# maxrmorrison/promonet

Hardware: AMD Instinct MI355X
Metric: audio samples/sec (22.05 kHz), batch-32 10 s utterances (higher is better)
Workload: dtype bf16; 1 GPU; Generator.forward (prepare_features + HiFi-GAN), batch 32 x 10 s per GPU (861 frames, 220416 samples each), random-init weights, bf16 MFMA operands, fp32 accumulate and activations; model=hifigan, batch_per_gpu=32, frames=861, devices=1, parallelism=batch-sharded x1

## Files before the change

include/promonet_hip.h:

```cpp
#ifndef PROMONET_HIP_H
#define PROMONET_HIP_H

#include <stddef.h>
#include <stdint.h>

#ifdef __cplusplus
extern "C" {
#endif

#define PM_OK 0
#define PM_EINVAL (-1)
#define PM_ESTATE (-2)
#define PM_EHIP (-3)
#define PM_ENOMEM (-4)
#define PM_ETIMEOUT (-5)

#define PM_F32 0
#define PM_F16 1
#define PM_BF16 2
#define PM_F16X3 3
#define PM_F16A2 4
#define PM_F16UX 5

#define PM_MAX_STAGES 8
// ... 100 lines not shown
                          int mode, float scale, void* workspace,
                          size_t workspace_bytes, void* stream);
int pm_block_cl(int dtype, const float* x_cl, float* out_cl,
                const float* const* w1, const float* const* b1,
                const float* const* w2, const float* const* b2,
                const int* dilations, int niter, int batch, int length,
                int channels, int kernel_size, int mode, float scale,
                void* workspace, size_t workspace_bytes, void* stream);
int pm_block_act16_cl(int dtype, int act_dtype, const float* x_cl,
                      float* out_cl, void* act16_cl, const float* const* w1,
                      const float* const* b1, const float* const* w2,
                      const float* const* b2, const int* dilations, int niter,
                      int batch, int length, int channels, int kernel_size,
                      int mode, float scale, void* workspace,
                      size_t workspace_bytes, void* stream);
int pm_mrf_cl(int dtype, const float* x_cl, float* out_cl,
              const float* const* w1, const float* const* b1,
              const float* const* w2, const float* const* b2,
              const int* dilations, int niter, int batch, int length,
              int channels, void* workspace, size_t workspace_bytes,
              void* stream);
int pm_input_conv_cl(int dtype, const float* x_cl, float* out_cl,
                     const float* weight, const float* bias,
                     const float* global_features,
                     const float* speaker_weight, const float* speaker_bias,
                     int global_batch, int global_channels, int batch,
                     int length, int c_in, int c_out, void* workspace,
                     size_t workspace_bytes, void* stream);
int pm_conv_transpose_cl(int dtype, const float* x_cl, float* out_cl,
                         const float* w, const float* bias, int batch,
                         int length, int c_in, int c_out, int rate, int lrelu,
                         void* workspace, size_t workspace_bytes,
                         void* stream);
int pm_conv_transpose_x16_cl(int dtype, const void* x16_cl, float* out_cl,
                             const float* w, const float* bias, int batch,
                             int length, int c_in, int c_out, int rate,
                             void* workspace, size_t workspace_bytes,
                             void* stream);
int pm_out_conv_tanh(const float* x_cl, const float* w, float* out,
                     int batch, int length, int channels, void* stream);
int pm_debug_timeline(void* dev_buffer);
int pm_debug_force(int walk_nseg, int upsample_groups);
int pm_debug_skew(int mode);
int pm_mfma_probe(int dtype, int iterations, const void* operands,
                  float* sink, int workgroups, void* stream);
size_t pm_walk_scratch_bytes(int batch);
int pm_fold_weight_norm(const float* g, const float* v, float* w, int rows,
                        int cols, void* stream);
int pm_to_channels_last(const float* src, float* dst, int batch, int channels,
                        int frames, int c_pad, void* stream);

int pm_grid_sample(const float* seq, const float* grid, float* out, int rows,
                   int n_in, int n_out, int mode, float scale, float offset,
                   float lo, float hi, void* stream);
int pm_stretch_grid(const float* ppg, int ppg_rows, const int* indices,
                    int n_indices, float* selected, float* grid, int frames,
                    int target_frames, void* stream);

#define PM_FARGAN_MIXED 16
typedef struct pm_fargan_s* pm_fargan_t;
int pm_fargan_create(int num_features, int global_channels, int weight_dtype,
                     pm_fargan_t* out);
int pm_fargan_destroy(pm_fargan_t h);
int pm_fargan_load_tensor(pm_fargan_t h, const char* name, const float* dev,
                          const int64_t* shape, int ndim, void* stream);
int pm_fargan_finalize(pm_fargan_t h, void* stream);
// ... 281 lines not shown
```

promonet_amd/_lib.py:

```python
import ctypes
import os
from pathlib import Path

import torch

LIB_PATH = Path(__file__).parent / 'lib' / 'libpromonet_hip.so'

PM_F32, PM_F16, PM_BF16, PM_F16X3, PM_F16A2, PM_F16UX = 0, 1, 2, 3, 4, 5
DTYPES = {'fp32': PM_F32, 'f32': PM_F32, 'f16': PM_F16, 'fp16': PM_F16,
          'bf16': PM_BF16, 'f16x3': PM_F16X3, 'f16a2': PM_F16A2,
          'f16ux': PM_F16UX,
          'mixed': 16}
MAX_STAGES, MAX_RESBLOCKS, MAX_DILATIONS = 8, 4, 4
SPARSE_METHODS = {None: 0, 'percentile': 1, 'constant': 2, 'topk': 3}
DISC_SPEC_R, DISC_SPEC_CMB, DISC_SPEC_DB = range(3)
FDISC_ACTIVATIONS = {'none': 0, 'relu': 1, 'sigmoid': 2}
(ADV_ABS_DIFF, ADV_SQ_ONE_MINUS, ADV_SQ, ADV_HINGE_ONE_MINUS,
 ADV_HINGE_ONE_PLUS) = range(5)
(OPTIM_MAX, OPTIM_MIN, OPTIM_MEAN, OPTIM_NORM, OPTIM_NORM_SQ, OPTIM_NONFINITE,
 OPTIM_FOUND_INF, OPTIM_INV_SCALE, OPTIM_COEF) = range(9)
OPTIM_STATS = 16

c_float_p = ctypes.c_void_p
c_int64_p = ctypes.POINTER(ctypes.c_int64)
# ... 21 lines not shown
    'pm_version': (_I, []),
    'pm_last_error': (ctypes.c_char_p, []),
    'pm_hifigan_create': (_I, [ctypes.POINTER(HifiganConfig),
                               ctypes.POINTER(_P)]),
    'pm_hifigan_destroy': (_I, [_P]),
    'pm_hifigan_load_tensor': (_I, [_P, ctypes.c_char_p, _P, c_int64_p, _I, _P]),
    'pm_hifigan_finalize': (_I, [_P, _P]),
    'pm_hifigan_workspace_bytes': (_S, [_P, _I, _I]),
    'pm_hifigan_hopsize': (_I, [_P]),
    'pm_hifigan_features_cl_channels': (_I, [_P]),
    'pm_hifigan_forward': (_I, [_P, _P, _P, _I, _P, _I, _I, _P, _S, _P]),
    'pm_hifigan_forward_cl': (_I, [_P, _P, _P, _I, _P, _I, _I, _P, _S, _P]),
    'pm_hifigan_forward_ragged': (_I, [_P, _P, _I, _P, _I, _P, _P, _I, _I, _P, _S, _P]),
    'pm_hifigan_context': (_I, [_P, ctypes.POINTER(_I), ctypes.POINTER(_I)]),
    'pm_hifigan_stream': (_I, [_P, _P, _I, _I, _P, _I, _I, _P, _P, _I, _I, _I,
                               _P, _I, _P, _S, _P]),
    'pm_hifigan_stream_workspace_bytes': (_S, [_P, _I, _I]),
    'pm_hifigan_profile_enable': (_I, [_P, _I]),
    'pm_hifigan_profile_only': (_I, [_P, ctypes.c_char_p]),
    'pm_hifigan_profile_collect': (_I, [_P]),
    'pm_hifigan_profile_reset': (_I, [_P]),
    'pm_hifigan_profile_report': (ctypes.c_char_p, [_P]),
    'pm_prepare_features': (_I, [_P] * 8 + [_I] * 9 + [_F] * 6 + [_P]),
    'pm_prepare_global_features': (_I, [_P] * 5 + [_I, _I, _I, _P]),
    'pm_prepare_global_features_linear': (_I, [_P] * 6 + [_I, _I, _I, _P]),
    'pm_op_workspace_bytes': (_S, [_I, _I, _I]),
    'pm_block_iteration_cl': (_I, [_I] + [_P] * 6 + [_I] * 6 + [_F, _P, _S, _P]),
    'pm_block_cl': (_I, [_I, _P, _P] + [_P] * 5 + [_I] * 6 + [_F, _P, _S, _P]),
    'pm_block_act16_cl': (
        _I, [_I, _I, _P, _P, _P] + [_P] * 5 + [_I] * 6 + [_F, _P, _S, _P]),
    'pm_mrf_cl': (_I, [_I, _P, _P] + [_P] * 5 + [_I] * 4 + [_P, _S, _P]),
    'pm_input_conv_cl': (_I, [_I] + [_P] * 7 + [_I] * 6 + [_P, _S, _P]),
    'pm_conv_transpose_cl': (_I, [_I] + [_P] * 4 + [_I] * 6 + [_P, _S, _P]),
    'pm_conv_transpose_x16_cl': (_I, [_I] + [_P] * 4 + [_I] * 5 + [_P, _S, _P]),
    'pm_out_conv_tanh': (_I, [_P, _P, _P, _I, _I, _I, _P]),
    'pm_debug_timeline': (_I, [_P]),
    'pm_debug_force': (_I, [_I, _I]),
    'pm_debug_skew': (_I, [_I]),
    'pm_mfma_probe': (_I, [_I, _I, _P, _P, _I, _P]),
    'pm_walk_scratch_bytes': (_S, [_I]),
    'pm_fold_weight_norm': (_I, [_P, _P, _P, _I, _I, _P]),
    'pm_to_channels_last': (_I, [_P, _P, _I, _I, _I, _I, _P]),
    'pm_grid_sample': (_I, [_P, _P, _P, _I, _I, _I, _I, _F, _F, _F, _F, _P]),
    'pm_stretch_grid': (_I, [_P, _I, _P, _I, _P, _P, _I, _I, _P]),
    'pm_fargan_create': (_I, [_I, _I, _I, ctypes.POINTER(_P)]),
    'pm_fargan_destroy': (_I, [_P]),
    'pm_fargan_load_tensor': (_I, [_P, ctypes.c_char_p, _P, c_int64_p, _I, _P]),
    'pm_fargan_finalize': (_I, [_P, _P]),
    'pm_fargan_workspace_bytes': (_S, [_P, _I, _I]),
    'pm_fargan_forward': (_I, [_P, _P, _I, _P, _I, _P, _I, _P, _I, _I, _P, _S, _P]),
    'pm_fargan_forward_ragged': (_I, [_P, _P, _I, _P, _I, _P, _I, _P, _P, _I, _I, _P, _S, _P]),
    'pm_fargan_forward_stateful': (_I, [_P, _P, _I, _P, _I, _P, _I, _P, _P, _P, _P, _I, _I, _P, _S, _P]),
    'pm_fargan_set_mode': (_I, [_P, _I]),
    'pm_fargan_check': (_I, [_P, _I, _I, _P, _P]),
    'pm_stft_scratch_bytes': (_S, [_I, _I]),
    'pm_stft_magnitude': (_I, [_P, _P, _I, _I, _P, _S, _P]),
    'pm_stft_magnitude_dft': (_I, [_P, _P, _I, _I, _P, _S, _P]),
    'pm_stft_mel_scratch_bytes': (_S, [_I]),
    'pm_stft_mel_prepare': (_I, [_P, _I, _P, _S, _P]),
    'pm_stft_mel': (_I, [_P, _P, _P, _I, _I, _I, _I, _F, _P]),
    'pm_stft_set_frames_per_group': (_I, [_I]),
    'pm_stft_set_loudness_passes': (_I, [_I]),
    'pm_stft_launch_info': (_I, [_I, _I, _I, ctypes.POINTER(_I), ctypes.POINTER(_I)]),
    'pm_linear_to_mel': (_I, [_P, _P, _P, _I, _I, _I, _I, _I, _F, _P]),
    'pm_stft_backward_scratch_bytes': (_S, [_I, _I]),
    'pm_stft_magnitude_backward': (_I, [_P, _P, _P, _I, _I, _P, _S, _P]),
# ... 137 lines not shown
```

promonet_amd/csrc/pm_api.hip:

```cpp
#include <hip/hip_runtime.h>

#include <algorithm>
#include <cstdarg>
#include <cstdio>
#include <cstring>
#include <map>
#include <mutex>
#include <string>
#include <vector>

#include "pm_host.h"
#include "pm_launch.h"
#include "pm_misc.h"

#define PM_VERSION 100

static thread_local char g_error[512] = "";

int pm_fail(int code, const char* fmt, ...) {
    va_list ap;
    va_start(ap, fmt);
    vsnprintf(g_error, sizeof(g_error), fmt, ap);
    va_end(ap);
    return code;
// ... 1187 lines not shown
    if (!x || !out || !w || !bias || !global || !ws_w || !ws_b || !ws)
        return pm_fail(PM_EINVAL, "null argument");
    if (gbatch != 1 && gbatch != B)
        return pm_fail(PM_EINVAL, "global batch must be 1 or batch");
    const int cop = pm_pad32(c_out);
    if (cop % 64 && cop != 32)
        return pm_fail(PM_EINVAL, "output channels %d unsupported", c_out);
    const InputConvLayout l = input_conv_layout(c_in, c_out, B, ws);
    if (ws_bytes < l.total)
        return pm_fail(PM_ENOMEM, "workspace too small");
    hipStream_t s = (hipStream_t)stream;
    Layer conv = input_layer(dtype, c_in, c_out);
    conv.w = l.w; conv.bias = l.bias;
    PM_HIP_TRY(pack_layer(conv, w, bias, s));
    PM_HIP_TRY(launch_speaker_bias(global, ws_w, ws_b, l.gbias, gbatch, G,
                                   c_out, s));
    PM_HIP_TRY(launch_input_conv(conv, x, out, l.gbias, gbatch, B, L, nullptr,
                                 s));
    return PM_OK;
}

struct TransposeLayout { float *w, *bias; size_t total; };
static TransposeLayout transpose_layout(int c_in, int c_out, int r,
                                        void* base) {
    const size_t ci = pm_pad32(c_in), co = pm_pad32(c_out);
    PmCarve c(base);
    float* w = c.take<float>(ci * co * 2 * r);
    c.take<float>(ci * co * 2 * r);
    return {w, c.take<float>(co * r), c.used};
}

static int conv_transpose_cl_impl(
    int dtype, const float* x, const void* x16, float* out, const float* w,
    const float* bias, int B, int L, int c_in, int c_out, int r, int lrelu,
    void* ws, size_t ws_bytes, void* stream) {
    if ((!x && !x16) || !out || !w || !bias || !ws)
        return pm_fail(PM_EINVAL, "null argument");
    if (r < 2 || (r & 1)) return pm_fail(PM_EINVAL, "rate %d unsupported", r);
    if (ws_bytes < pm_op_workspace_bytes(c_in, c_out, 2 * r))
        return pm_fail(PM_ENOMEM, "workspace too small");
    const TransposeLayout l = transpose_layout(c_in, c_out, r, ws);
    if (l.total > pm_op_workspace_bytes(c_in, c_out, 2 * r))
        return pm_fail(PM_ESTATE, "the layout outgrew its public bound");
    hipStream_t s = (hipStream_t)stream;
    Layer up = upsample_layer(dtype, c_in, c_out, r);
    if (x16 && !takes_x16(up))
        return pm_fail(PM_EINVAL, "a 16-bit operand input needs a 16-bit "
                       "operand type and the narrow upsampler kernel");
    up.w = l.w; up.bias = l.bias;
    PM_HIP_TRY(pack_layer(up, w, bias, s));
    PM_HIP_TRY(launch_upsample(up, x, x16, out, lrelu, B, L, nullptr, 1, s));
    return PM_OK;
}

extern "C" int pm_conv_transpose_cl(
    int dtype, const float* x, float* out, const float* w, const float* bias,
    int B, int L, int c_in, int c_out, int r, int lrelu, void* ws,
    size_t ws_bytes, void* stream) {
    if (!x) return pm_fail(PM_EINVAL, "null argument");
    return conv_transpose_cl_impl(dtype, x, nullptr, out, w, bias, B, L, c_in,
                                  c_out, r, lrelu, ws, ws_bytes, stream);
}

extern "C" int pm_conv_transpose_x16_cl(
    int dtype, const void* x16, float* out, const float* w, const float* bias,
    int B, int L, int c_in, int c_out, int r, void* ws, size_t ws_bytes,
    void* stream) {
    if (!x16) return pm_fail(PM_EINVAL, "null argument");
    return conv_transpose_cl_impl(dtype, nullptr, x16, out, w, bias, B, L, c_in,
                                  c_out, r, 1, ws, ws_bytes, stream);
}

extern "C" int pm_out_conv_tanh(
    const float* x, const float* w, float* out, int B, int L, int C,
    void* stream) {
    if (!x || !w || !out) return pm_fail(PM_EINVAL, "null argument");
    if (pm_pad32(C) > 64)
        return pm_fail(PM_EINVAL, "channels %d unsupported", C);
    PM_HIP_TRY(launch_out_conv(x, w, out, B, L, C, nullptr, 1,
                               (hipStream_t)stream));
    return PM_OK;
}

static bool debug_hooks_enabled() {
    static const bool enabled = [] {
        const char* e = getenv("PROMONET_HIP_DEBUG");
        return e && e[0] == '1';
    }();
    return enabled;
}

extern "C" int pm_debug_force(int walk_nseg, int upsample_groups) {
    if (!debug_hooks_enabled())
        return pm_fail(PM_ESTATE, "debug hooks are disabled "
                       "(start the process with PROMONET_HIP_DEBUG=1)");
    if (walk_nseg < 0 || upsample_groups < 0)
        return pm_fail(PM_EINVAL, "negative value");
    pm_force().walk_nseg = walk_nseg;
    pm_force().upsample_groups = upsample_groups;
    return PM_OK;
}

extern "C" int pm_mfma_probe(int dtype, int iterations, const void* operands,
// ... 92 lines not shown
```

promonet_amd/csrc/pm_common.h:

```cpp
#pragma once
#include <hip/hip_runtime.h>
#include <stdint.h>

#define PM_LRELU_SLOPE 0.1f

typedef float floatx16 __attribute__((ext_vector_type(16)));
typedef unsigned int pm_u4 __attribute__((ext_vector_type(4)));
typedef _Float16 half8 __attribute__((ext_vector_type(8)));
typedef _Float16 half4 __attribute__((ext_vector_type(4)));
typedef __bf16 bf16x8 __attribute__((ext_vector_type(8)));
typedef __bf16 bf16x4 __attribute__((ext_vector_type(4)));

__device__ __forceinline__ float pm_lrelu(float v) {
    return __builtin_fmaxf(v, v * PM_LRELU_SLOPE);
}
typedef float pm_f4 __attribute__((ext_vector_type(4)));
__device__ __forceinline__ float4 pm_lrelu4(float4 v) {
    pm_f4 w = {v.x, v.y, v.z, v.w};
    w = __builtin_elementwise_max(w, w * PM_LRELU_SLOPE);
    return make_float4(w.x, w.y, w.z, w.w);
}

#define PM_ELEM_COMMON(bias_split)                                            \
    static constexpr bool BIAS_SPLIT = bias_split;                            \
// ... 196 lines not shown
    typedef ElemF16X3::frag_t bfrag_t;
    typedef afrag_t frag_t;
    static constexpr int ESZ = 4;
    static constexpr int WSZ = 2;
    static constexpr int ID = 4;
    static constexpr bool SPLIT = true;
    static constexpr bool BIAS_SPLIT = true;
    __device__ static __forceinline__ void mma(
        const afrag_t& a, const bfrag_t& b, floatx16& c) {
        c = __builtin_amdgcn_mfma_f32_32x32x16_f16(a, b.lo, c, 0, 0, 0);
        c = __builtin_amdgcn_mfma_f32_32x32x16_f16(a, b.hi, c, 0, 0, 0);
    }
    __device__ static __forceinline__ void store4_at(
        char* rowp, int ch, float4 v) {
        ElemF16X3::store4_at(rowp, ch, v);
    }
    __device__ static __forceinline__ void pack_store(
        void* out, long long index, float v) {
        reinterpret_cast<_Float16*>(out)[index] = (_Float16)v;
    }
    __device__ static __forceinline__ lds_t cvt(float v) { return (_Float16)v; }
    __device__ static __forceinline__ void mma_bias(
        const afrag_t& a, floatx16& c) {
        ElemF16::mma_bias(a, c);
    }
};

__device__ __forceinline__ void pm_block_sync() {
    __builtin_amdgcn_fence(__ATOMIC_RELEASE, "workgroup", "local");
    __builtin_amdgcn_s_barrier();
    __builtin_amdgcn_fence(__ATOMIC_ACQUIRE, "workgroup", "local");
}

__device__ __forceinline__ int pm_xcd_remap(int bid, int nwg) {
    const int xcd = bid & 7;
    const int q = nwg >> 3, r = nwg & 7;
    const int base = xcd < r ? xcd * (q + 1) : r * (q + 1) + (xcd - r) * q;
    return base + (bid >> 3);
}
```

promonet_amd/csrc/pm_conv.h:

```cpp
#pragma once
#include <type_traits>

#include "pm_common.h"


template <class ET, int CH, int NT, int XR_MAX>
struct ChunkStager {
    static constexpr int Q = CH / 4;
    static constexpr int MAXIT = (XR_MAX * Q + NT - 1) / NT;
    static constexpr int S = CH * ET::ESZ + 16;
    float4 r[MAXIT];

    __device__ __forceinline__ void load(
        const float* __restrict__ xb, int cstride, int c0, int t_first,
        int XR, int L, int tid) {
        const int lo = max(t_first, 0);
        const int hi = min(L, t_first + XR);
        const __amdgpu_buffer_rsrc_t rsrc = __builtin_amdgcn_make_buffer_rsrc(
            const_cast<float*>(xb) + (size_t)lo * cstride, 0,
            max(hi - lo, 0) * cstride * 4, 0x00020000);
#pragma unroll
        for (int it = 0; it < MAXIT; ++it) {
            const int idx = tid + it * NT;
            const int row = idx / Q, q = idx % Q;
// ... 597 lines not shown
                                              acc[mt][nt][4 * g4 + 2] * scale);
                        r.w = __float_as_uint(__uint_as_float(o.w) +
                                              acc[mt][nt][4 * g4 + 3] * scale);
                        __builtin_amdgcn_raw_buffer_store_b128(
                            r, orsrc, voff + g4 * 32, 0, 0);
                    }
                }
            }
    } else {
        const float s = mode == 1 ? scale : 1.f;
#pragma unroll
        for (int mt = 0; mt < MTW; ++mt)
#pragma unroll
            for (int nt = 0; nt < NTW; ++nt) {
                const unsigned voff =
                    voff0 + (unsigned)((mt * 32 + nt * 32 * C) * 4);
#pragma unroll
                for (int g4 = 0; g4 < 4; ++g4) {
                    pm_u4 r;
                    r.x = __float_as_uint(acc[mt][nt][4 * g4 + 0] * s);
                    r.y = __float_as_uint(acc[mt][nt][4 * g4 + 1] * s);
                    r.z = __float_as_uint(acc[mt][nt][4 * g4 + 2] * s);
                    r.w = __float_as_uint(acc[mt][nt][4 * g4 + 3] * s);
                    __builtin_amdgcn_raw_buffer_store_b128(
                        r, orsrc, voff + g4 * 32, 0, 0);
                }
            }
    }
    PM_STAMP(a, 5);
    PM_STAMP_WALL(a, blockIdx.x, 13);
}


struct SingleArgs {
    const void* x16;
    const float* x;
    float* out;
    const void* w;
    const float* bias;
    const float* gbias;
    int gbias_batch;
    int B, L, Cin, M;
    int Lout;
    int bins;
    unsigned* maxbits;
    const float* grad;
    int lrelu;
    int pad;
    int phase_c, phase_p, phase_r;
    int ntiles, nmblocks;
    const int* lengths;
    int len_scale;
};

__device__ __forceinline__ unsigned pm_float_order_bits(float f) {
    const unsigned u = __float_as_uint(f);
    return (u & 0x80000000u) ? ~u : (u | 0x80000000u);
}

template <class ET, int KT, int KSPAN, int CH, int WM, int WN, int MTW, int NTW,
          int EPI>
__global__ __launch_bounds__(WM * WN * 64) void conv_single_kernel(
    SingleArgs a) {
    typedef typename ET::afrag_t frag_t;
    constexpr int KC = CH / 16;
    constexpr int N1 = WN * NTW * 32;
// ... 57 lines not shown
    const frag_t* w = reinterpret_cast<const frag_t*>(a.w) +
                      (size_t)(m0 / 32) * w_mt_stride + lane;
    frag_t afirst[G][MTW];
    load_a_group<ET, MTW, G>(afirst, w, w_mt_stride);
    const int lane_off_x =
        ((wn * NTW * 32) + ln + js) * SX + lh * 8 * ET::ESZ;

#pragma unroll 1
    for (int c = 0; c < NCH; ++c) {
        char* cur = smem + (c & 1) * XR * SX;
        if (c + 1 < NCH) {
            if (pre) stager.load16(xb16, Cin, (c + 1) * CH, t_first, XR, L, tid);
            else stager.load(xb, Cin, (c + 1) * CH, t_first, XR, L, tid);
        }
        mma_taps<ET, KT, KC, MTW, NTW, G, SX>(
            acc, cur + lane_off_x, SX, w + (size_t)c * (KT * KC * 64),
            w_mt_stride, afirst,
            c + 1 < NCH ? w + (size_t)(c + 1) * (KT * KC * 64) : nullptr);
        if (c + 1 < NCH) {
            char* nxt = smem + ((c + 1) & 1) * XR * SX;
            if (pre) stager.store16(nxt, XR, tid);
            else if (a.lrelu) stager.template store<true>(nxt, XR, tid);
            else stager.template store<false>(nxt, XR, tid);
            pm_block_sync();
        }
    }

    if constexpr (EPI == 0) {
    const float* gb = a.gbias
        ? a.gbias + (size_t)(a.gbias_batch == 1 ? 0 : b) * M : nullptr;
    const __amdgpu_buffer_rsrc_t orsrc = __builtin_amdgcn_make_buffer_rsrc(
        a.out + ((size_t)b * a.Lout + t0) * M, 0,
        min(Lout - t0, N1) * M * 4, 0x00020000);
#pragma unroll
    for (int mt = 0; mt < MTW; ++mt) {
        const int co_base = m0 + mt * 32 + 4 * lh;
        float4 bias[4];
#pragma unroll
        for (int g4 = 0; g4 < 4; ++g4) {
            const int co = co_base + 8 * g4;
            bias[g4] = *reinterpret_cast<const float4*>(a.bias + co);
            if (gb) {
                const float4 g = *reinterpret_cast<const float4*>(gb + co);
                bias[g4].x += g.x; bias[g4].y += g.y;
                bias[g4].z += g.z; bias[g4].w += g.w;
            }
        }
#pragma unroll
        for (int nt = 0; nt < NTW; ++nt) {
            const int n = (wn * NTW + nt) * 32 + ln;
            const unsigned voff = (unsigned)((n * M + co_base) * 4);
#pragma unroll
            for (int g4 = 0; g4 < 4; ++g4) {
                pm_u4 r;
                r.x = __float_as_uint(acc[mt][nt][4 * g4 + 0] + bias[g4].x);
                r.y = __float_as_uint(acc[mt][nt][4 * g4 + 1] + bias[g4].y);
                r.z = __float_as_uint(acc[mt][nt][4 * g4 + 2] + bias[g4].z);
                r.w = __float_as_uint(acc[mt][nt][4 * g4 + 3] + bias[g4].w);
                __builtin_amdgcn_raw_buffer_store_b128(
                    r, orsrc, voff + g4 * 32, 0, 0);
            }
        }
    }
    } else if constexpr (EPI == 3) {
    float* ob = a.out + (size_t)b * a.Lout * M;
    const float* gb = a.grad + (size_t)b * a.bins * a.Lout;
#pragma unroll
    for (int mt = 0; mt < MTW; ++mt) {
        const int row_base = m0 + mt * 32 + 4 * lh;
#pragma unroll
        for (int nt = 0; nt < NTW; ++nt) {
            const int n = (wn * NTW + nt) * 32 + ln;
            const int t = t0 + n;
            if (t < a.Lout) {
#pragma unroll
                for (int g4 = 0; g4 < 4; ++g4) {
                    float v[4];
#pragma unroll
                    for (int pr = 0; pr < 2; ++pr) {
                        const int bin = (row_base + 8 * g4) / 2 + pr;
                        const float re = acc[mt][nt][4 * g4 + 2 * pr];
                        const float im = acc[mt][nt][4 * g4 + 2 * pr + 1];
                        float scale = 0.f;
                        if (bin < a.bins)
                            scale = gb[(size_t)bin * a.Lout + t] /
                                    sqrtf(re * re + im * im + 1e-6f);
                        v[2 * pr] = scale * re;
                        v[2 * pr + 1] = scale * im;
                    }
                    *reinterpret_cast<float4*>(
                        ob + (size_t)t * M + row_base + 8 * g4) =
                        make_float4(v[0], v[1], v[2], v[3]);
                }
            }
        }
// ... 10 lines not shown
            const int t = t0 + n;
#pragma unroll
            for (int g4 = 0; g4 < 4; ++g4) {
#pragma unroll
                for (int pr = 0; pr < 2; ++pr) {
                    const int bin = (row_base + 8 * g4) / 2 + pr;
                    const float re = acc[mt][nt][4 * g4 + 2 * pr];
                    const float im = acc[mt][nt][4 * g4 + 2 * pr + 1];
                    const float pw = re * re + im * im;
                    if (t < a.Lout && bin < a.bins) {
                        float v;
                        if constexpr (EPI == 1) {
                            v = sqrtf(pw + 1e-6f);
                        } else {
                            v = 10.f * log10f(fmaxf(1e-10f, pw));
                            local_max = fmaxf(local_max, v);
                        }
                        ob[(size_t)bin * a.Lout + t] = v;
                    }
                }
            }
        }
    }
    if constexpr (EPI == 2) {
#pragma unroll
        for (int o = 32; o > 0; o >>= 1)
            local_max = fmaxf(local_max, __shfl_xor(local_max, o, 64));
        if (lane == 0 && local_max > -INFINITY)
            atomicMax(a.maxbits + b, pm_float_order_bits(local_max));
    }
    }
}

template <class ET, int CIN, int WM, int WN, int MTW, int NTW>
__global__ __launch_bounds__(WM * WN * 64) void conv_upsample_kernel(
    SingleArgs a) {
    typedef typename ET::afrag_t frag_t;
    constexpr int KT = 2, KSPAN = 3;
    constexpr int KC = CIN / 16;
    constexpr int N1 = WN * NTW * 32;
    constexpr int NT = WM * WN * 64;
    constexpr int S = CIN * ET::ESZ + 16;
    constexpr int XR = N1 + KSPAN - 1;
    constexpr int MB = WM * MTW * 32;
    constexpr int G = 4;
    constexpr int SLAB = 128;

    extern __shared__ __attribute__((aligned(16))) char smem[];

    const int tid = threadIdx.x;
    const int lane = tid & 63;
    const int wave = __builtin_amdgcn_readfirstlane(tid >> 6);
    const int wm = wave / WN, wn = wave % WN;
    const int ln = lane & 31, lh = lane >> 5;

    const int wg = pm_xcd_remap(blockIdx.x, gridDim.x);
    const int mg = wg % a.nmblocks;
    const int tile = (wg / a.nmblocks) % a.ntiles;
    const int b = wg / (a.nmblocks * a.ntiles);
    const int t0 = tile * N1;
    const int M = a.M;
    const int L = a.lengths ? min(a.lengths[b] * a.len_scale, a.L) : a.L;
    const int Lout = a.lengths ? L : a.Lout;
    if (t0 >= Lout) return;

    const float* xb = a.x + (size_t)b * a.L * CIN;
    const int t_first = t0 - a.pad;
// ... 12 lines not shown

    constexpr int w_mt_stride = KT * KC * 64;
    const int per_group = (M / MB) / a.nmblocks;
    const frag_t* wbase = reinterpret_cast<const frag_t*>(a.w) + lane;
    const float* gb = a.gbias
        ? a.gbias + (size_t)(a.gbias_batch == 1 ? 0 : b) * M : nullptr;
    const __amdgpu_buffer_rsrc_t orsrc = __builtin_amdgcn_make_buffer_rsrc(
        a.out + ((size_t)b * a.Lout + t0) * M, 0,
        min(Lout - t0, N1) * M * 4, 0x00020000);

    frag_t afirst[G][MTW];
    load_a_group<ET, MTW, G>(
        afirst,
        wbase + (size_t)((mg * per_group * MB + wm * MTW * 32) / 32) * w_mt_stride,
        w_mt_stride);
#pragma unroll 1
    for (int mi = 0; mi < per_group; ++mi) {
        const int m0 = (mg * per_group + mi) * MB + wm * MTW * 32;
        const int js =
            (a.phase_r > 0 && (m0 / a.phase_c) + a.phase_p >= a.phase_r) ? 1 : 0;
        const frag_t* w = wbase + (size_t)(m0 / 32) * w_mt_stride;
        floatx16 acc[MTW][NTW];
#pragma unroll
        for (int mt = 0; mt < MTW; ++mt)
#pragma unroll
            for (int nt = 0; nt < NTW; ++nt)
#pragma unroll
                for (int r = 0; r < 16; ++r) acc[mt][nt][r] = 0.f;
        const int lane_off =
            ((wn * NTW * 32) + ln + js) * S + lh * 8 * ET::ESZ;
        mma_taps<ET, KT, KC, MTW, NTW, G, S>(
            acc, smem + lane_off, S, w, w_mt_stride, afirst,
            mi + 1 < per_group ? w + (size_t)(MB / 32) * w_mt_stride : nullptr);
#pragma unroll
        for (int mt = 0; mt < MTW; ++mt) {
            const int co_base = m0 + mt * 32 + 4 * lh;
            float4 bias[4];
#pragma unroll
            for (int g4 = 0; g4 < 4; ++g4) {
                const int co = co_base + 8 * g4;
                bias[g4] = *reinterpret_cast<const float4*>(a.bias + co);
                if (gb) {
                    const float4 g = *reinterpret_cast<const float4*>(gb + co);
                    bias[g4].x += g.x; bias[g4].y += g.y;
                    bias[g4].z += g.z; bias[g4].w += g.w;
                }
            }
#pragma unroll
            for (int nt = 0; nt < NTW; ++nt) {
                const int n = (wn * NTW + nt) * 32 + ln;
                const unsigned voff = (unsigned)((n * M + co_base) * 4);
#pragma unroll
                for (int g4 = 0; g4 < 4; ++g4) {
                    pm_u4 r;
                    r.x = __float_as_uint(acc[mt][nt][4 * g4 + 0] + bias[g4].x);
                    r.y = __float_as_uint(acc[mt][nt][4 * g4 + 1] + bias[g4].y);
                    r.z = __float_as_uint(acc[mt][nt][4 * g4 + 2] + bias[g4].z);
                    r.w = __float_as_uint(acc[mt][nt][4 * g4 + 3] + bias[g4].w);
                    __builtin_amdgcn_raw_buffer_store_b128(
                        r, orsrc, voff + g4 * 32, 0, 0);
                }
            }
        }
    }
}


struct Block3Args {
    const float* x;
    float* out;
    const void* w1[3];
    const void* w2[3];
    int dil[3];
    int niter;
    int B, L;
    int mode;
    float scale;
    int ntiles, halo, TL;
    const int* lengths;
    int len_scale;
    void* act16;
    int act16_type;
    PM_TIMELINE_FIELD
};

template <class ET, int C, int K, int WM, int WN, int NTW>
__host__ __device__ constexpr int block3_smem_bytes() {
    constexpr int NC = WN * NTW * 32;
    constexpr int S = C * ET::ESZ + 16;
    return (NC + 10 * ((K - 1) / 2)) * S + (NC + (K - 1)) * S;
}

struct B3Walk {
    int b;
    int L;
// ... 1565 lines not shown
```

promonet_amd/csrc/pm_fft.h:

```cpp
#pragma once
#include "pm_common.h"

#define PM_FFT_N 1024
#define PM_FFT_HOP 256
#define PM_FFT_BINS 513
#define PM_FFT_PAD 384
#define PM_FFT_TAB_W512 1024
#define PM_FFT_TAB_W1024 (1024 + 1024)
#define PM_FFT_TAB_FLOATS (1024 + 1024 + 1026)
#define PM_DB_PER_LOG2 3.01029995663981195f
#ifdef PM_FFT_LIBM_SQRT
#define PM_FFT_SQRT(x) sqrtf(x)
#else
#define PM_FFT_SQRT(x) __builtin_amdgcn_sqrtf(x)
#endif

struct FftArgs {
    const float* audio;
    float* out;
    const float* tables;
    float* group_max;
    float* group_min;
    const float* weights;
    const int* mel_span;
// ... 54 lines not shown
    PM_DPP_ADD(0x4E, 0xf);
    PM_DPP_ADD(0x141, 0xf);
    PM_DPP_ADD(0x140, 0xf);
    PM_DPP_ADD(0x142, 0xa);
    PM_DPP_ADD(0x143, 0xc);
#undef PM_DPP_ADD
    return __builtin_bit_cast(float, __builtin_amdgcn_readlane(
        __builtin_bit_cast(int, v), 63));
}
__device__ __forceinline__ float pk_norm(pm_v2 a) {
    const pm_v2 q = a * a;
    return q.x + q.y;
}

__device__ __forceinline__ void pm_radix8(pm_v2 (&a)[8]) {
    const float h = 0.70710678118654752440f;
    const pm_v2 b0 = pk_add(a[0], a[4]), b4 = pk_sub(a[0], a[4]);
    const pm_v2 b1 = pk_add(a[1], a[5]), e5 = pk_sub(a[1], a[5]);
    const pm_v2 b2 = pk_add(a[2], a[6]), e6 = pk_sub(a[2], a[6]);
    const pm_v2 b3 = pk_add(a[3], a[7]), e7 = pk_sub(a[3], a[7]);
    {
        const pm_v2 d0 = pk_add(b0, b2), d1 = pk_sub(b0, b2);
        const pm_v2 d2 = pk_add(b1, b3), e = pk_sub(b1, b3);
        a[0] = pk_add(d0, d2); a[2] = pk_sub_i(d1, e);
        a[4] = pk_sub(d0, d2); a[6] = pk_add_i(d1, e);
    }
    {
        const pm_v2 u5 = pk_sub_i(e5, e5), u7 = pk_add_i(e7, e7);
        const pm_v2 d0 = pk_sub_i(b4, e6), d1 = pk_add_i(b4, e6);
        const pm_v2 d2 = pk_sub(u5, u7) * h, e = pk_add(u5, u7) * h;
        a[1] = pk_add(d0, d2); a[3] = pk_sub_i(d1, e);
        a[5] = pk_sub(d0, d2); a[7] = pk_add_i(d1, e);
    }
}

__device__ __forceinline__ void pm_wave_lds_sync() {
    __builtin_amdgcn_fence(__ATOMIC_RELEASE, "wavefront", "local");
    __builtin_amdgcn_wave_barrier();
    __builtin_amdgcn_fence(__ATOMIC_ACQUIRE, "wavefront", "local");
}

#define PM_FFT_MEL_CAP 2048
template <int EPI, int NW, int FPW>
__host__ __device__ constexpr int pm_fft_smem_bytes() {
    constexpr int FR = NW * FPW;
    return NW * 576 * 8 +
           (EPI == 2 ? 64 : EPI == 5 ? 8 * (FR + 1) * 4 : EPI == 6 ? 8 * (FR + 1) * 4 + 128
                     : PM_FFT_BINS * (FR + 1) * 4) +
           (EPI == 4 ? PM_FFT_MEL_CAP * 4 : 0);
}

__device__ __forceinline__ void pm_fft_load_frame(
    pm_v2 (&raw)[8], const float* __restrict__ ab, int t, int N, int lane) {
    const int base = t * PM_FFT_HOP - PM_FFT_PAD;
    if (base >= 0 && base + PM_FFT_N <= N) {
        const float* p = ab + base + 2 * lane;
        if ((reinterpret_cast<uintptr_t>(p) & 7) == 0) {
#pragma unroll
            for (int i = 0; i < 8; ++i)
                raw[i] = *reinterpret_cast<const pm_v2*>(p + 128 * i);
        } else {
#pragma unroll
            for (int i = 0; i < 8; ++i)
                raw[i] = pm_v2{p[128 * i], p[128 * i + 1]};
        }
    } else {
#pragma unroll
        for (int i = 0; i < 8; ++i) {
            float v[2];
#pragma unroll
            for (int e = 0; e < 2; ++e) {
                int j = base + 2 * (64 * i + lane) + e;
// ... 416 lines not shown
```

promonet_amd/csrc/pm_launch.h:

```cpp
#pragma once
#include <algorithm>
#include <cstdlib>
#include <cstring>
#include <map>
#include <mutex>
#include <utility>

#include "pm_conv.h"
#include "pm_host.h"

struct PmForce { int walk_nseg = 0; int upsample_groups = 0; int skew = 0; };
#define PM_SKEW_WG_SCRATCH (256 << 10)
inline PmForce& pm_force() { static thread_local PmForce f; return f; }

inline bool pm_narrow_allowed() {
#ifdef PM_TUNING
    static const bool allowed = !getenv("PM_NO_NARROW");
    return allowed;
#else
    return true;
#endif
}

inline int pm_fusion_level() {
#ifdef PM_TUNING
    static const int level = [] {
        const char* e = getenv("PM_FUSION");
        return (e && !strcmp(e, "pair")) ? 0 : (e && !strcmp(e, "block")) ? 1 : 2;
    }();
    return level;
#else
    return 2;
#endif
}

#define PM_LDS_BYTES (160 * 1024)

template <class ET, int C> struct PairCfg;
template <> struct PairCfg<ElemF16, 256> { enum { WM = 8, WN = 1, NTW = 6, CH = 64, ALIAS = 1 }; };
template <> struct PairCfg<ElemF16, 128> { enum { WM = 4, WN = 2, NTW = 4, CH = 64, ALIAS = 0 }; };
template <> struct PairCfg<ElemF16, 64>  { enum { WM = 2, WN = 2, NTW = 2, CH = 64, ALIAS = 0 }; };
template <> struct PairCfg<ElemF16, 32>  { enum { WM = 1, WN = 4, NTW = 1, CH = 32, ALIAS = 0 }; };
template <int C> struct PairCfg<ElemBF16, C> : PairCfg<ElemF16, C> {};
template <> struct PairCfg<ElemF32, 256> { enum { WM = 4, WN = 2, NTW = 2, CH = 64, ALIAS = 1 }; };
template <> struct PairCfg<ElemF32, 128> { enum { WM = 4, WN = 2, NTW = 3, CH = 64, ALIAS = 1 }; };
template <> struct PairCfg<ElemF32, 64>  { enum { WM = 2, WN = 2, NTW = 1, CH = 64, ALIAS = 0 }; };
template <> struct PairCfg<ElemF32, 32>  { enum { WM = 1, WN = 4, NTW = 1, CH = 32, ALIAS = 0 }; };
template <int C> struct PairCfg<ElemF16X3, C> : PairCfg<ElemF32, C> {};
template <int C> struct PairCfg<ElemF16A2, C> : PairCfg<ElemF32, C> {};

template <class ET, int C> struct PairCfgNarrow : PairCfg<ET, C> {};
template <> struct PairCfgNarrow<ElemF16, 256> { enum { WM = 8, WN = 1, NTW = 2, CH = PairCfg<ElemF16, 256>::CH, ALIAS = 1 }; };
template <> struct PairCfgNarrow<ElemF16, 128> { enum { WM = 4, WN = 2, NTW = 2, CH = PairCfg<ElemF16, 128>::CH, ALIAS = 0 }; };
template <> struct PairCfgNarrow<ElemF32, 256> { enum { WM = 4, WN = 2, NTW = 1, CH = 64, ALIAS = 0 }; };
template <> struct PairCfgNarrow<ElemF32, 128> { enum { WM = 4, WN = 2, NTW = 1, CH = 64, ALIAS = 0 }; };
template <> struct PairCfgNarrow<ElemF16X3, 256> : PairCfgNarrow<ElemF32, 256> {};
template <> struct PairCfgNarrow<ElemF16X3, 128> : PairCfgNarrow<ElemF32, 128> {};
template <> struct PairCfgNarrow<ElemF16A2, 256> : PairCfgNarrow<ElemF32, 256> {};
template <> struct PairCfgNarrow<ElemF16A2, 128> : PairCfgNarrow<ElemF32, 128> {};
template <> struct PairCfgNarrow<ElemBF16, 256> : PairCfgNarrow<ElemF16, 256> {};
template <> struct PairCfgNarrow<ElemBF16, 128> : PairCfgNarrow<ElemF16, 128> {};
#define PM_NARROW_BELOW 150

template <class ET, int C> constexpr bool pm_one_packing_c() {
    return PairCfg<ET, C>::CH == (C < 64 ? C : 64) &&
           PairCfgNarrow<ET, C>::CH == PairCfg<ET, C>::CH;
}
template <class ET> constexpr bool pm_one_packing() {
    return pm_one_packing_c<ET, 32>() &&
// ... 511 lines not shown
            case 3: return launch_single_cfg<ET, KT, KSPAN, 64, 4, 2, 1, 2>(a, s);
            case 5:
                if constexpr (KT == 2)
                    return launch_single_cfg<ET, KT, KSPAN, 64, 4, 2, 1, 4>(a, s);
                break;
        }
    } else if (ch == 32) {
        switch (cfg) {
            case 1: return launch_single_cfg<ET, KT, KSPAN, 32, 2, 2, 1, 2>(a, s);
            case 2: return launch_single_cfg<ET, KT, KSPAN, 32, 1, 4, 1, 1>(a, s);
        }
    }
    return hipErrorInvalidValue;
}

template <class ET, int CIN>
static hipError_t launch_upsample_cfg(const SingleArgs& a0, hipStream_t stream) {
    if constexpr (ET::ESZ != 2) {
        return hipErrorNotSupported;
    } else {
    constexpr int WM = 4, WN = 2, MTW = 2, NTW = 2;
    constexpr int N1 = WN * NTW * 32, MB = WM * MTW * 32;
    SingleArgs a = a0;
    if (a.Cin != CIN || a.M % MB) return hipErrorInvalidValue;
    a.ntiles = (a.Lout + N1 - 1) / N1;
    const int mblocks = a.M / MB;
    int groups = 1;
    while (groups < mblocks && (long long)a.ntiles * a.B * groups < 512)
        groups *= 2;
    if (pm_force().upsample_groups > 0) groups = pm_force().upsample_groups;
    if (groups > mblocks) groups = mblocks;
    while (mblocks % groups) groups /= 2;
    a.nmblocks = groups;
    auto kern = conv_upsample_kernel<ET, CIN, WM, WN, MTW, NTW>;
    constexpr int smem = (N1 + 2) * (CIN * ET::ESZ + 16);
    hipError_t e = pm_ensure_dynamic_lds(
        reinterpret_cast<const void*>(kern), smem);
    if (e != hipSuccess) return e;
    hipLaunchKernelGGL(kern, dim3(a.ntiles * a.nmblocks * a.B),
                       dim3(WM * WN * 64), smem, stream, a);
    return hipGetLastError();
    }
}

template <class ET>
hipError_t pm_launch_single(
    int kind, int ch, int cfg, const SingleArgs& a, hipStream_t s) {
    if (kind == 1 && cfg == 4) {
        if (ch == 256) return launch_upsample_cfg<ET, 256>(a, s);
        if (ch == 512) return launch_upsample_cfg<ET, 512>(a, s);
        return hipErrorInvalidValue;
    }
    if (kind == 0) return launch_single_k<ET, 7, 7>(ch, cfg, a, s);
    if (kind == 1) return launch_single_k<ET, 2, 3>(ch, cfg, a, s);
    return hipErrorInvalidValue;
}

#ifdef PM_INSTANTIATE_STFT
hipError_t pm_launch_stft(int epi, const SingleArgs& a, hipStream_t s) {
    if (epi == 1)
        return launch_single_cfg<ElemF32, 4, 4, 64, 2, 2, 1, 2, 1>(a, s);
    if (epi == 3)
        return launch_single_cfg<ElemF32, 4, 4, 64, 2, 2, 1, 2, 3>(a, s);
    if (epi == 0)
        return launch_single_cfg<ElemF32, 4, 4, 64, 2, 2, 1, 2, 0>(a, s);
    return hipErrorInvalidValue;
}
#endif

#endif
```

Before: 390.4 million samples/s.

## Stage conv epilogue through LDS for full-row coalesced output stores

Adds an epilogue that transposes MFMA accumulators through a per-wave, XOR-swizzled LDS buffer so each lane writes contiguous 16-byte chunks of whole output rows, adding bias, with a cache-policy aux flag. It is used in the single-conv kernel (bf16, KT=2, MTW=1) and in the upsample kernel, which gets extra LDS per wave (CP 32 or 8 depending on budget). The aim is to replace scattered channel-strided global stores with coalesced row stores. In exchange the upsample kernel uses more LDS, which can lower occupancy, and adds wave-level syncs. A ragged conv-transpose API entry is also added.

```diff
diff --git a/include/promonet_hip.h b/include/promonet_hip.h
--- a/include/promonet_hip.h
+++ b/include/promonet_hip.h
@@ -156,6 +156,12 @@
                          int length, int c_in, int c_out, int rate, int lrelu,
                          void* workspace, size_t workspace_bytes,
                          void* stream);
+int pm_conv_transpose_ragged_cl(int dtype, const float* x_cl, float* out_cl,
+                                const float* w, const float* bias,
+                                const int* lengths, int batch, int length,
+                                int c_in, int c_out, int rate, int lrelu,
+                                void* workspace, size_t workspace_bytes,
+                                void* stream);
 int pm_conv_transpose_x16_cl(int dtype, const void* x16_cl, float* out_cl,
                              const float* w, const float* bias, int batch,
                              int length, int c_in, int c_out, int rate,
diff --git a/promonet_amd/_lib.py b/promonet_amd/_lib.py
--- a/promonet_amd/_lib.py
+++ b/promonet_amd/_lib.py
@@ -77,6 +77,8 @@
     'pm_mrf_cl': (_I, [_I, _P, _P] + [_P] * 5 + [_I] * 4 + [_P, _S, _P]),
     'pm_input_conv_cl': (_I, [_I] + [_P] * 7 + [_I] * 6 + [_P, _S, _P]),
     'pm_conv_transpose_cl': (_I, [_I] + [_P] * 4 + [_I] * 6 + [_P, _S, _P]),
+    'pm_conv_transpose_ragged_cl': (
+        _I, [_I] + [_P] * 5 + [_I] * 6 + [_P, _S, _P]),
     'pm_conv_transpose_x16_cl': (_I, [_I] + [_P] * 4 + [_I] * 5 + [_P, _S, _P]),
     'pm_out_conv_tanh': (_I, [_P, _P, _P, _I, _I, _I, _P]),
     'pm_debug_timeline': (_I, [_P]),
diff --git a/promonet_amd/csrc/pm_api.hip b/promonet_amd/csrc/pm_api.hip
--- a/promonet_amd/csrc/pm_api.hip
+++ b/promonet_amd/csrc/pm_api.hip
@@ -1243,8 +1243,8 @@
 
 static int conv_transpose_cl_impl(
     int dtype, const float* x, const void* x16, float* out, const float* w,
-    const float* bias, int B, int L, int c_in, int c_out, int r, int lrelu,
-    void* ws, size_t ws_bytes, void* stream) {
+    const float* bias, int B, int L, const int* lengths, int c_in, int c_out,
+    int r, int lrelu, void* ws, size_t ws_bytes, void* stream) {
     if ((!x && !x16) || !out || !w || !bias || !ws)
         return pm_fail(PM_EINVAL, "null argument");
     if (r < 2 || (r & 1)) return pm_fail(PM_EINVAL, "rate %d unsupported", r);
@@ -1260,7 +1260,7 @@
                        "operand type and the narrow upsampler kernel");
     up.w = l.w; up.bias = l.bias;
     PM_HIP_TRY(pack_layer(up, w, bias, s));
-    PM_HIP_TRY(launch_upsample(up, x, x16, out, lrelu, B, L, nullptr, 1, s));
+    PM_HIP_TRY(launch_upsample(up, x, x16, out, lrelu, B, L, lengths, 1, s));
     return PM_OK;
 }
 
@@ -1269,8 +1269,19 @@
     int B, int L, int c_in, int c_out, int r, int lrelu, void* ws,
     size_t ws_bytes, void* stream) {
     if (!x) return pm_fail(PM_EINVAL, "null argument");
-    return conv_transpose_cl_impl(dtype, x, nullptr, out, w, bias, B, L, c_in,
-                                  c_out, r, lrelu, ws, ws_bytes, stream);
+    return conv_transpose_cl_impl(dtype, x, nullptr, out, w, bias, B, L,
+                                  nullptr, c_in, c_out, r, lrelu, ws, ws_bytes,
+                                  stream);
+}
+
+extern "C" int pm_conv_transpose_ragged_cl(
+    int dtype, const float* x, float* out, const float* w, const float* bias,
+    const int* lengths, int B, int L, int c_in, int c_out, int r, int lrelu,
+    void* ws, size_t ws_bytes, void* stream) {
+    if (!x || !lengths) return pm_fail(PM_EINVAL, "null argument");
+    return conv_transpose_cl_impl(dtype, x, nullptr, out, w, bias, B, L,
+                                  lengths, c_in, c_out, r, lrelu, ws, ws_bytes,
+                                  stream);
 }
 
 extern "C" int pm_conv_transpose_x16_cl(
@@ -1278,8 +1289,9 @@
     int B, int L, int c_in, int c_out, int r, void* ws, size_t ws_bytes,
     void* stream) {
     if (!x16) return pm_fail(PM_EINVAL, "null argument");
-    return conv_transpose_cl_impl(dtype, nullptr, x16, out, w, bias, B, L, c_in,
-                                  c_out, r, 1, ws, ws_bytes, stream);
+    return conv_transpose_cl_impl(dtype, nullptr, x16, out, w, bias, B, L,
+                                  nullptr, c_in, c_out, r, 1, ws, ws_bytes,
+                                  stream);
 }
 
 extern "C" int pm_out_conv_tanh(
diff --git a/promonet_amd/csrc/pm_common.h b/promonet_amd/csrc/pm_common.h
--- a/promonet_amd/csrc/pm_common.h
+++ b/promonet_amd/csrc/pm_common.h
@@ -252,6 +252,12 @@
     __builtin_amdgcn_fence(__ATOMIC_ACQUIRE, "workgroup", "local");
 }
 
+__device__ __forceinline__ void pm_wave_lds_sync() {
+    __builtin_amdgcn_fence(__ATOMIC_RELEASE, "wavefront", "local");
+    __builtin_amdgcn_wave_barrier();
+    __builtin_amdgcn_fence(__ATOMIC_ACQUIRE, "wavefront", "local");
+}
+
 __device__ __forceinline__ int pm_xcd_remap(int bid, int nwg) {
     const int xcd = bid & 7;
     const int q = nwg >> 3, r = nwg & 7;
diff --git a/promonet_amd/csrc/pm_conv.h b/promonet_amd/csrc/pm_conv.h
--- a/promonet_amd/csrc/pm_conv.h
+++ b/promonet_amd/csrc/pm_conv.h
@@ -653,6 +653,74 @@
 }
 
 
+#ifndef PM_ROWS_AUX
+#define PM_ROWS_AUX 2
+#endif
+#ifndef PM_SINGLE_ROWS
+#define PM_SINGLE_ROWS 1
+#endif
+template <int MTW, int CP>
+struct RowStores {
+    static constexpr int RUN = MTW * 32 * 4;
+    static constexpr int WAVE = CP * RUN;
+    static constexpr int LPR = RUN / 16;
+    static constexpr int CPI = 64 / LPR;
+    static_assert(MTW == 1 || MTW == 2, "8 or 16 slots of 16 bytes");
+    static_assert(CP == 8 || CP == 16 || CP == 32, "whole 8-lane store groups");
+    static __device__ __forceinline__ int at(int col, int s) {
+        return col * RUN + ((s ^ (col & 7)) << 4);
+    }
+};
+
+template <int MTW, int NTW, int CP>
+__device__ __forceinline__ void pm_store_rows(
+    const floatx16 (&acc)[MTW][NTW], char* ebuf, const float* bias_ptr,
+    const float* gb, __amdgpu_buffer_rsrc_t orsrc, int M, int m0, int n0,
+    int lane) {
+    typedef RowStores<MTW, CP> R;
+    const int ln = lane & 31, lh = lane >> 5;
+    const int q = lane % R::LPR, h = lane / R::LPR;
+    const int co = m0 + 4 * q;
+    float4 bias = *reinterpret_cast<const float4*>(bias_ptr + co);
+    if (gb) {
+        const float4 g = *reinterpret_cast<const float4*>(gb + co);
+        bias.x += g.x; bias.y += g.y; bias.z += g.z; bias.w += g.w;
+    }
+#pragma unroll
+    for (int pass = 0; pass < NTW * (32 / CP); ++pass) {
+        const int nt = pass / (32 / CP), sub = pass % (32 / CP);
+        pm_wave_lds_sync();
+        if (CP == 32 || ln / CP == sub) {
+#pragma unroll
+            for (int mt = 0; mt < MTW; ++mt)
+#pragma unroll
+                for (int g4 = 0; g4 < 4; ++g4)
+                    *reinterpret_cast<float4*>(
+                        ebuf + R::at(ln % CP, mt * 8 + 2 * g4 + lh)) =
+                        make_float4(acc[mt][nt][4 * g4 + 0],
+                                    acc[mt][nt][4 * g4 + 1],
+                                    acc[mt][nt][4 * g4 + 2],
+                                    acc[mt][nt][4 * g4 + 3]);
+        }
+        pm_wave_lds_sync();
+        const int n = n0 + nt * 32 + sub * CP + h;
+        const unsigned voff = (unsigned)((n * M + co) * 4);
+#pragma unroll
+        for (int k = 0; k < CP / R::CPI; ++k) {
+            const float4 v = *reinterpret_cast<const float4*>(
+                ebuf + R::at(R::CPI * k + h, q));
+            pm_u4 r;
+            r.x = __float_as_uint(v.x + bias.x);
+            r.y = __float_as_uint(v.y + bias.y);
+            r.z = __float_as_uint(v.z + bias.z);
+            r.w = __float_as_uint(v.w + bias.w);
+            __builtin_amdgcn_raw_buffer_store_b128(
+                r, orsrc, voff + (unsigned)(k * R::CPI * M * 4), 0,
+                PM_ROWS_AUX);
+        }
+    }
+}
+
 struct SingleArgs {
     const void* x16;
     const float* x;
@@ -776,6 +844,15 @@
     const __amdgpu_buffer_rsrc_t orsrc = __builtin_amdgcn_make_buffer_rsrc(
         a.out + ((size_t)b * a.Lout + t0) * M, 0,
         min(Lout - t0, N1) * M * 4, 0x00020000);
+    constexpr bool ROWS =
+        PM_SINGLE_ROWS && ET::ESZ == 2 && KT == 2 && MTW == 1 &&
+        WM * WN * 32 * 128 <= 2 * XR * SX;
+    if constexpr (ROWS) {
+        pm_block_sync();
+        pm_store_rows<MTW, NTW, 32>(
+            acc, smem + wave * RowStores<MTW, 32>::WAVE, a.bias, gb, orsrc, M,
+            m0, wn * NTW * 32, lane);
+    } else {
 #pragma unroll
     for (int mt = 0; mt < MTW; ++mt) {
         const int co_base = m0 + mt * 32 + 4 * lh;
@@ -805,6 +882,7 @@
                     r, orsrc, voff + g4 * 32, 0, 0);
             }
         }
+    }
     }
     } else if constexpr (EPI == 3) {
     float* ob = a.out + (size_t)b * a.Lout * M;
@@ -881,7 +959,7 @@
     }
 }
 
-template <class ET, int CIN, int WM, int WN, int MTW, int NTW>
+template <class ET, int CIN, int WM, int WN, int MTW, int NTW, int ROWS = 0>
 __global__ __launch_bounds__(WM * WN * 64) void conv_upsample_kernel(
     SingleArgs a) {
     typedef typename ET::afrag_t frag_t;
@@ -960,6 +1038,11 @@
         mma_taps<ET, KT, KC, MTW, NTW, G, S>(
             acc, smem + lane_off, S, w, w_mt_stride, afirst,
             mi + 1 < per_group ? w + (size_t)(MB / 32) * w_mt_stride : nullptr);
+        if constexpr (ROWS) {
+            pm_store_rows<MTW, NTW, ROWS>(
+                acc, smem + XR * S + wave * RowStores<MTW, ROWS>::WAVE, a.bias,
+                gb, orsrc, M, m0, wn * NTW * 32, lane);
+        } else {
 #pragma unroll
         for (int mt = 0; mt < MTW; ++mt) {
             const int co_base = m0 + mt * 32 + 4 * lh;
@@ -989,6 +1072,7 @@
                         r, orsrc, voff + g4 * 32, 0, 0);
                 }
             }
+        }
         }
     }
 }
diff --git a/promonet_amd/csrc/pm_fft.h b/promonet_amd/csrc/pm_fft.h
--- a/promonet_amd/csrc/pm_fft.h
+++ b/promonet_amd/csrc/pm_fft.h
@@ -110,12 +110,6 @@
         a[1] = pk_add(d0, d2); a[3] = pk_sub_i(d1, e);
         a[5] = pk_sub(d0, d2); a[7] = pk_add_i(d1, e);
     }
-}
-
-__device__ __forceinline__ void pm_wave_lds_sync() {
-    __builtin_amdgcn_fence(__ATOMIC_RELEASE, "wavefront", "local");
-    __builtin_amdgcn_wave_barrier();
-    __builtin_amdgcn_fence(__ATOMIC_ACQUIRE, "wavefront", "local");
 }
 
 #define PM_FFT_MEL_CAP 2048
diff --git a/promonet_amd/csrc/pm_launch.h b/promonet_amd/csrc/pm_launch.h
--- a/promonet_amd/csrc/pm_launch.h
+++ b/promonet_amd/csrc/pm_launch.h
@@ -35,6 +35,10 @@
 }
 
 #define PM_LDS_BYTES (160 * 1024)
+
+#ifndef PM_UPSAMPLE_ROWS
+#define PM_UPSAMPLE_ROWS 1
+#endif
 
 template <class ET, int C> struct PairCfg;
 template <> struct PairCfg<ElemF16, 256> { enum { WM = 8, WN = 1, NTW = 6, CH = 64, ALIAS = 1 }; };
@@ -612,13 +616,27 @@
     if (groups > mblocks) groups = mblocks;
     while (mblocks % groups) groups /= 2;
     a.nmblocks = groups;
+    constexpr int xtile = (N1 + 2) * (CIN * ET::ESZ + 16);
+    const dim3 grid(a.ntiles * a.nmblocks * a.B), block(WM * WN * 64);
+    constexpr int CP =
+        xtile + WM * WN * RowStores<MTW, 32>::WAVE <= PM_LDS_BYTES ? 32 : 8;
+    if constexpr (PM_UPSAMPLE_ROWS &&
+                  xtile + WM * WN * RowStores<MTW, CP>::WAVE <= PM_LDS_BYTES) {
+        if (pm_force().upsample_groups == 0) {
+            auto rows = conv_upsample_kernel<ET, CIN, WM, WN, MTW, NTW, CP>;
+            constexpr int smem = xtile + WM * WN * RowStores<MTW, CP>::WAVE;
+            hipError_t e = pm_ensure_dynamic_lds(
+                reinterpret_cast<const void*>(rows), smem);
+            if (e != hipSuccess) return e;
+            hipLaunchKernelGGL(rows, grid, block, smem, stream, a);
+            return hipGetLastError();
+        }
+    }
     auto kern = conv_upsample_kernel<ET, CIN, WM, WN, MTW, NTW>;
-    constexpr int smem = (N1 + 2) * (CIN * ET::ESZ + 16);
     hipError_t e = pm_ensure_dynamic_lds(
-        reinterpret_cast<const void*>(kern), smem);
+        reinterpret_cast<const void*>(kern), xtile);
     if (e != hipSuccess) return e;
-    hipLaunchKernelGGL(kern, dim3(a.ntiles * a.nmblocks * a.B),
-                       dim3(WM * WN * 64), smem, stream, a);
+    hipLaunchKernelGGL(kern, grid, block, xtile, stream, a);
     return hipGetLastError();
     }
 }
```

After: 394.4 million samples/s (median of 6 runs). 1.0% higher.
